# snsinfu/2022a-genome-dynamics

Hardware: AMD Instinct MI355X
Metric: bead-steps/sec on 100kb whole-genome model, 1 GPU and 8-GPU replica farm (higher is better)
Workload: dtype f32

## Files before the change

### 2022a-genome-dynamics_amd/__init__.py

```python
from __future__ import annotations

import ctypes as C
import os
from dataclasses import dataclass

import numpy as np

_HERE = os.path.dirname(os.path.abspath(__file__))
LIBGDYN_PATH = os.path.join(_HERE, "csrc", "libgdyn.so")

GD_BOX_OPEN, GD_BOX_PERIODIC = 0, 1
POT_HARMONIC, POT_SPRING, POT_SEMISPRING, POT_SOFTCORE = 0, 1, 2, 3
NOISE_PHILOX, NOISE_ZERO, NOISE_HOST, NOISE_MT19937 = 0, 1, 2, 3
RUN_UPDATE_SCALES, RUN_WALL_DYNAMICS, RUN_DEFER_CALLBACK, RUN_COMPENSATED, RUN_UNCOMPENSATED = 1, 2, 4, 8, 16
ALL_REPLICAS = 0xffffffff
ABI_VERSION = 5
TERM_PAIR, TERM_BOND, TERM_BEND, TERM_POINT, TERM_WALL, TERM_DYNAMIC, TERM_ALL = 1, 2, 4, 8, 16, 32, 63

_STATUS = {1: "GD_EINVAL", 2: "GD_ENODEVICE", 3: "GD_EHIP", 4: "GD_ENOMEM", 5: "GD_ESTATE", 6: "GD_EUNSUPPORTED"}


class GdynError(RuntimeError):
    def __init__(self, code, msg):
        super().__init__(f"{_STATUS.get(code, code)}: {msg}")
# ... 330 lines not shown

    def set_tuning(self, skin=0.0, rebuild_interval=0, adapt_interval=1, list_width=0, kernel_path=0, near_fraction=0.0, auto_skin=0):
        t = Tuning(skin, rebuild_interval, adapt_interval, list_width, kernel_path, near_fraction, auto_skin)
        self.lib.check(self.lib.dll.gd_set_tuning(self._h, C.byref(t)))

    def _groups_fn(self, name):
        f = getattr(self.lib.dll, name, None)
        if f is None:
            raise GdynError(6, f"{name}: not in this library (include/gdyn_groups.h: csrc/libgdyn.so only)")
        return f

    def set_step_groups(self, mode=0):
        f = self._groups_fn("gd_set_step_groups")
        f.argtypes = [C.c_void_p, C.c_uint32]
        self.lib.check(f(self._h, mode))

    def step_groups(self):
        f = self._groups_fn("gd_get_step_groups")
        f.argtypes = [C.c_void_p, C.POINTER(C.c_uint32), C.POINTER(C.c_uint32)]
        mode, last = C.c_uint32(0), C.c_uint32(0)
        self.lib.check(f(self._h, C.byref(mode), C.byref(last)))
        return mode.value, last.value

    def timing(self):
        t = Timing()
        self.lib.check(self.lib.dll.gd_get_timing(self._h, C.byref(t)))
        return t

    def debug_bench(self, what, n=20):
        f = getattr(self.lib.dll, "gd_debug_bench", None)
        if f is None:
            raise GdynError(6, "gd_debug_bench: not in this library (developer builds only: make -C csrc dev; load('libgdyn_dev.so'))")
        f.argtypes = [C.c_void_p, C.c_int, C.c_int, C.POINTER(C.c_double)]
        ms = C.c_double(0)
        self.lib.check(f(self._h, what, n, C.byref(ms)))
        return ms.value

    def stream(self):
        p = C.c_void_p()
        self.lib.check(self.lib.dll.gd_get_stream(self._h, C.byref(p)))
        return p.value
```

### 2022a-genome-dynamics_amd/csrc/gdyn_capi.hip

```cpp
#include <algorithm>
#include <cmath>
#include <cstdio>
#include <cstdlib>
#include <cstring>
#include <new>
#include <string>
#include <vector>

#include <hip/hip_fp16.h>

#include "gdyn_system.hpp"
#include "gdyn_once.hpp"
#ifdef GD_DEV
#include "gdyn_dev.h"
#endif


static thread_local char g_err[1024];
extern "C" const char *gd_last_error(void) { return g_err; }
int gd_report_error(int code, const char *msg)
{
    snprintf(g_err, sizeof g_err, "%s", msg);
    return code;
}
// ... 40 lines not shown
    if (s->R % GD_XCDS == 0 && !dev_env("GDYN_SLICE_MAP")) s->cpb = 0;
    s->ens.reset(s->N, s->R); s->mob.assign(s->N, 1.0); s->bend.assign(s->N, 0.0);
    s->hctx.assign(s->R, DevCtx{});
    for (auto &c : s->hctx) { c.bead_scale = 1; c.bond_scale = 1; }
    s->rp.reset(s->N, s->R);
    s->lcount.assign(2 * (size_t)s->R, 0ull);
    s->ncell_cap = (uint32_t)std::min<uint64_t>(std::max<uint64_t>(8ull * s->N, 4096ull), 262144ull);
    if (const char *e = dev_env("GDYN_NEAR_FRAC")) s->near_frac = atof(e);
    if (const char *e = dev_env("GDYN_SKIN")) { s->pol.skin = atof(e); s->pol.skin_fixed = true; }
    if (dev_env("GDYN_AUTO_SKIN")) s->pol.tuner.enabled = true;
    if (const char *e = dev_env("GDYN_TILE_CAPS")) { auto &c = s->pol.tile_caps; c.clear(); for (const char *q = e; *q;) { c.push_back((unsigned)strtoul(q, (char **)&q, 10)); if (*q == ',') q++; } }
    if (const char *e = dev_env("GDYN_K_TARGET")) s->pol.k_target = atof(e);
    if (dev_env("GDYN_DEBUG")) s->pol.trace = stderr;
    size_t free_b = 0, total_b = 0;
    if (hipMemGetInfo(&free_b, &total_b) == hipSuccess) s->pol.mem_total = total_b;
    hipError_t e = hipStreamCreateWithFlags(&s->stream, hipStreamNonBlocking);
    if (e != hipSuccess) { delete s; return fail(GD_EHIP, "hipStreamCreate failed: %s", hipGetErrorString(e)); }
    const size_t RNp = (size_t)s->R * s->Np, RN = (size_t)s->R * s->N;
    bool ok = true;
    for (int k = 0; k < 2; k++) {
        ok = ok && s->pos[k].resize(RNp) == hipSuccess && s->orig[k].resize(RNp) == hipSuccess && s->ctx[k].resize(s->R) == hipSuccess &&
             s->react_part[k].resize((size_t)s->R * s->nblk) == hipSuccess;
    }
    ok = ok && s->xb.resize(RNp) == hipSuccess && s->slot_of.resize(RN) == hipSuccess && s->bbox_enc.resize((size_t)2 * s->R * 6) == hipSuccess && s->bbox_w.resize((size_t)s->R * s->nblk * (GD_BLOCK / 64) * 6) == hipSuccess &&
         s->rank.resize(RNp) == hipSuccess && s->members.resize(RNp) == hipSuccess && s->cell_cnt.resize((size_t)s->R * (s->ncell_cap + 1)) == hipSuccess &&
         s->cell_start.resize((size_t)s->R * (s->ncell_cap + 1)) == hipSuccess && s->meta.resize(RNp) == hipSuccess &&
         s->flags.resize((size_t)s->R * GD_NFLAGS) == hipSuccess && s->bbox.resize((size_t)s->R * s->nblk * 6) == hipSuccess &&
         s->ab.resize(RNp) == hipSuccess && s->mobs.resize(RNp) == hipSuccess && s->grid.resize(s->R) == hipSuccess &&
         s->epart.resize((size_t)s->R * s->nblk) == hipSuccess &&
         s->lcount_d.resize(2 * (size_t)s->R) == hipSuccess && s->dmax.resize((size_t)s->R * GD_DMAX_STRIDE) == hipSuccess && s->fout.resize(RN) == hipSuccess && s->snap.resize(RN) == hipSuccess &&
         s->tiles.resize((size_t)s->R * s->nblk) == hipSuccess &&
         s->rec_x0.resize(RNp) == hipSuccess && s->rec_mo.resize(RNp) == hipSuccess && s->len_prev.resize((size_t)s->R * s->N) == hipSuccess &&
         s->wtab.resize(RNp / 64) == hipSuccess && s->need_prev.resize((size_t)s->R * s->N) == hipSuccess && s->pool.resize(4) == hipSuccess && s->rqueue.resize(RNp / 64) == hipSuccess &&
         s->lo.resize(RN) == hipSuccess;
    s->lo_valid = ok;
    if (!ok) { delete s; return fail(GD_ENOMEM, "gd_create: device allocation failed (%zu slots)", RNp); }
    gd_launch_identity(s->orig[0].p, s->slot_of.p, s->N, s->Np, s->R, s->stream);
    if (hipStreamSynchronize(s->stream) != hipSuccess) { delete s; return fail(GD_EHIP, "gd_create: identity kernel failed"); }
    *out = s;
    return GD_OK;
}

extern "C" int gd_destroy(gd_system *s)
{
    if (!s) return GD_OK;
    (void)hipSetDevice(s->device);
// ... 292 lines not shown
    if (t->near_fraction < 0 || t->near_fraction > 1) return fail(GD_EINVAL, "gd_set_tuning: near_fraction must be in [0,1]");
    HIPCHK(hipSetDevice(s->device));
    if (s->pol.set_tuning(t->skin, t->rebuild_interval, t->adapt_interval, t->list_width, t->auto_skin != 0 || dev_env("GDYN_AUTO_SKIN")))
        (void)s->nbr.resize(0);
    if (t->near_fraction > 0) s->near_frac = t->near_fraction;
    s->kernel_path = t->kernel_path;
    s->list.drop();
    return GD_OK;
}
extern "C" int gd_get_timing(gd_system *s, gd_timing *o) { if (!s || !o) return fail(GD_EINVAL, "gd_get_timing: NULL"); *o = s->timing; return GD_OK; }
extern "C" int gd_groups_abi_version(void) { return GD_GROUPS_ABI_VERSION; }
extern "C" int gd_set_step_groups(gd_system *s, uint32_t mode)
{
    if (!s) return fail(GD_EINVAL, "gd_set_step_groups: NULL system");
    if (mode > gd::STEP_GROUPS_TWO) return fail(GD_EINVAL, "gd_set_step_groups: mode must be 0 (rule), 1 (one launch) or 2 (two groups wherever results allow)");
    s->group_mode = mode;
    return GD_OK;
}
extern "C" int gd_get_step_groups(gd_system *s, uint32_t *mode, uint32_t *last_groups)
{
    if (!s) return fail(GD_EINVAL, "gd_get_step_groups: NULL system");
    if (mode) *mode = s->group_mode;
    if (last_groups) *last_groups = s->groups_last;
    return GD_OK;
}
extern "C" int gd_get_stream(gd_system *s, void **st) { if (!s || !st) return fail(GD_EINVAL, "gd_get_stream: NULL"); *st = (void *)s->stream; return GD_OK; }


static float pair_cutoff(const gd_system *s)
{
    double m = 0;
    if (s->has_pair) {
        if (s->pair.eps_a != 0 && s->pair.sigma_a > m) m = s->pair.sigma_a;
        if (s->pair.eps_b != 0 && s->pair.sigma_b > m) m = s->pair.sigma_b;
    }
    return (float)m;
}

static int finalize_topology(gd_system *s)
{
    if (!s->topo_dirty) return GD_OK;
    HIPCHK(hipSetDevice(s->device));
    const uint32_t N = s->N;
    std::vector<gd_bond_params> types = s->btypes;
    std::vector<int> terms = s->bterm;
    std::vector<Bond> all = s->bonds;
// ... 418 lines not shown
        q.scaling.from_host = 1;
        q.scaling.bead_next = scale_at(s, s->bs_init, s->bs_tau, time);
        q.scaling.bond_next = scale_at(s, s->bo_init, s->bo_tau, time);
    };
    size_t nev = 0;
    HIPCHK(hipEventRecord(get_event(s, nev++), s->stream));
    int64_t k = 0;
    c.on_search_list = s->list.valid && s->list.search_list;
    while (k < chunk) {
        if (!s->list.valid || s->list.steps_since_build >= s->pol.K) {
            s->pol.take_pending_skin(pair_cutoff(s));
            hipEvent_t e1 = get_event(s, nev++);
            GDCHK(enqueue_build(s, list_radius(s, run, (uint32_t)(k + s->pol.K)), with_list));
            s->list.enter_use(false);
            HIPCHK(hipEventRecord(e1, s->stream));
            c.spans.push_back({nev - 1, 1});
        }
        const int64_t n = std::min<int64_t>((int64_t)s->pol.K - s->list.steps_since_build, chunk - k);
        hipEvent_t e1 = get_event(s, nev++);
        uint32_t min_blocks = gd::STEP_GROUPS_MIN_BLOCKS, a16 = gd::STEP_GROUPS_A16;
        if (const char *e = dev_env("GDYN_GROUP_MIN_BLOCKS")) min_blocks = (uint32_t)atoi(e);
        if (const char *e = dev_env("GDYN_GROUP_A16")) a16 = (uint32_t)atoi(e);
        const uint32_t ra = gd::step_group_split(s->group_mode, group_state(s, host_noise), min_blocks, a16);
        if (ra) { GDCHK(fork_groups(s)); s->groups_last = 2; }
        for (int64_t q = 0; q < n; q++) {
            fill_common(s, p);
            p.dt_d = run->timestep; p.dt = (float)run->timestep; p.kT = (float)run->temperature; p.seed = run->seed;
            p.seeds = run->replica_seeds ? s->seeds_d.p : nullptr;
            p.noise_mode = run->noise_mode; p.run_flags = run->flags; p.comp = comp ? 1 : 0;
            p.host_noise = host_noise ? s->noise.p + (size_t)(done + k + q) * RN * 3 : nullptr;
            host_scales(p, k + q);
            p.record_disp = (s->list.steps_since_build + (uint32_t)q + 1u == s->pol.K);
            c.full_interval |= p.record_disp != 0;
            if (ra) {
                p.r0 = 0; p.nrep = ra; gd_launch_step(p, GD_MODE_STEP, s->stream);
                p.r0 = ra; p.nrep = s->R - ra; gd_launch_step(p, GD_MODE_STEP, s->stream2);
            } else gd_launch_step(p, GD_MODE_STEP, s->stream);
            if (s->sw.n) launch_softwell(s, p, 0);
            if (s->rp.any()) launch_replica_pairs(s, p, 0);
            s->pcur ^= 1; s->ccur ^= 1;
        }
        if (ra) GDCHK(join_groups(s));
        HIPCHK(hipEventRecord(e1, s->stream));
        c.spans.push_back({nev - 1, 0});
        s->timing.step_launches += (uint64_t)n;
        s->list.stepped((uint32_t)n);
        k += n;
    }
    const bool defer = (run->flags & GD_RUN_DEFER_CALLBACK) && done + chunk == run->steps;
    if (!defer) {
        fill_common(s, p);
        p.dt_d = run->timestep; p.dt = (float)run->timestep; p.run_flags = run->flags;
        host_scales(p, chunk);
        gd_launch_finalize(p, 0, s->stream);
        s->ccur ^= 1;
    } else {
        s->pend_dt = run->timestep; s->pend_flags = run->flags;
        if (s->has_wall) {
            fill_common(s, p);
// ... 50 lines not shown
    return GD_OK;
}

extern "C" int gd_run(gd_system *s, const gd_run_desc *run)
{
    if (!s || !run) return fail(GD_EINVAL, "gd_run: NULL argument");
    if (run->spacestep != 0) return fail(GD_EUNSUPPORTED, "gd_run: spacestep != 0 (adaptive timestep) is not supported");
    if (run->steps < 0 || !(run->timestep > 0) || run->temperature < 0) return fail(GD_EINVAL, "gd_run: bad steps/timestep/temperature");
    if (run->noise_mode < 0 || run->noise_mode > GD_NOISE_HOST)
        return fail(run->noise_mode == 3 ? GD_EUNSUPPORTED : GD_EINVAL, "gd_run: noise_mode %d not available on the device", run->noise_mode);
    if (run->noise_mode == GD_NOISE_HOST && !run->host_noise) return fail(GD_EINVAL, "gd_run: host noise requested without array");
    if ((run->flags & GD_RUN_WALL_DYNAMICS) && !s->has_wall) return fail(GD_ESTATE, "gd_run: wall dynamics requested without a wall");
    if ((run->flags & GD_RUN_UPDATE_SCALES) && !s->has_scaling) return fail(GD_ESTATE, "gd_run: scale updates requested without gd_set_scaling");
    GDCHK(prepare(s));
    GDCHK(apply_pending(s));
    s->state_serial++;
    if (run->timestep != s->last_dt || run->temperature != s->last_kT) { s->pol.a2_ema = 0; s->last_dt = run->timestep; s->last_kT = run->temperature; }
    if (s->pol.adapt && s->pol.K > 4 && ((run->flags ^ s->last_flags) & (GD_RUN_WALL_DYNAMICS | GD_RUN_UPDATE_SCALES)) != 0 && s->rebuilds > 0)
        s->pol.K -= s->pol.K / 5;
    s->last_flags = run->flags;
    const bool with_list = pair_cutoff(s) > 0;
    const size_t RN = (size_t)s->R * s->N;
    memset(&s->timing, 0, sizeof s->timing);
    s->groups_last = 1;

    const bool host_noise = run->noise_mode == GD_NOISE_HOST && run->temperature > 0;
    if (host_noise) {
        const size_t n = (size_t)run->steps * RN * 3;
        std::vector<float> h(n);
        for (size_t i = 0; i < n; i++) h[i] = (float)run->host_noise[i];
        HIPCHK(s->noise.resize(n, false));
        HIPCHK(hipMemcpy(s->noise.p, h.data(), n * sizeof(float), hipMemcpyHostToDevice));
    }

    const bool comp = run->steps > 0 && want_compensated(s, run);
    if (comp) {
        if (!s->lo_valid) { HIPCHK(hipMemsetAsync(s->lo.p, 0, RN * sizeof(float4), s->stream)); s->lo_valid = true; }
        HIPCHK(s->snap_lo.resize(RN, false));
    }
    if (run->steps > 0) s->comp_last = comp;
    if (run->steps > 0 && !comp) s->lo_valid = false;

    if (run->replica_seeds) {
        static_assert(sizeof(unsigned long long) == sizeof(uint64_t), "seed width");
        HIPCHK(s->seeds_d.resize(s->R, false));
        HIPCHK(hipMemcpy(s->seeds_d.p, run->replica_seeds, s->R * sizeof(uint64_t), hipMemcpyHostToDevice));
    }
// ... 178 lines not shown
```

### 2022a-genome-dynamics_amd/csrc/gdyn_kernels.hip

```cpp
#include <hip/hip_fp16.h>

#include <algorithm>

#include "gdyn_types.h"

#include "gdyn_stamps.h"

#if GD_ABL == 40 || GD_ABL == 41 || GD_ABL == 43
#define GD_REPLAY 1
constexpr bool RP_MEM = (GD_ABL == 40), RP_ALU = (GD_ABL == 41 || GD_ABL == 43);
#define GD_CONSUME4(v) asm volatile("" :: "v"((v).x), "v"((v).y), "v"((v).z), "v"((v).w))
#define GD_LAUNDER4(v) asm volatile("" : "+v"((v).x), "+v"((v).y), "+v"((v).z), "+v"((v).w))
#endif

#define TERM_PAIR 1u
#define TERM_BOND 2u
#define TERM_BEND 4u
#define TERM_POINT 8u
#define TERM_WALL 16u
#define TERM_DYNAMIC 32u
#define RUN_UPDATE_SCALES 1
#define RUN_WALL_DYNAMICS 2
#define NOISE_PHILOX 0
#define NOISE_ZERO 1
// ... 404 lines not shown
__device__ __forceinline__ float integrate(const StepParams &p, const CtxF &s_ctx, const StepBead &bead, unsigned r, unsigned blk,
                                           float mu, const float3 &z, const float3 &F, float disp2)
{
    const float3 xi = bead.xi;
    const float mu_dt = mu * p.dt;
    const float sg = s_ctx.sg_uniform >= 0.f ? s_ctx.sg_uniform : sqrtf(2.0f * p.kT * mu_dt);
    const float ex = mu_dt * F.x + sg * z.x, ey = mu_dt * F.y + sg * z.y, ez = mu_dt * F.z + sg * z.z;
    float nx = xi.x + ex, ny = xi.y + ey, nz = xi.z + ez;
    if (p.comp) {
        float4 *lp = p.lo + ((size_t)r * p.N + bead.oid);
        const float4 l = *lp;
        const float tx = l.x + ex, ty = l.y + ey, tz = l.z + ez;
        nx = xi.x + tx; ny = xi.y + ty; nz = xi.z + tz;
        const float bx = nx - xi.x, by = ny - xi.y, bz = nz - xi.z;
        *lp = make_float4((xi.x - (nx - bx)) + (tx - bx), (xi.y - (ny - by)) + (ty - by), (xi.z - (nz - bz)) + (tz - bz), 0.f);
    }
    if (TILED) *(float4 *)((char *)(p.pos_out + bead.rbase + (size_t)blk * GD_BLOCK) + bead.local * 16u) = make_float4(nx, ny, nz, bead.xi4.w);
    else p.pos_out[bead.g] = make_float4(nx, ny, nz, bead.xi4.w);
    float dnew2 = 0.f;
    if (TILED) { const float e2 = ex * ex + ey * ey + ez * ez; dnew2 = (disp2 + e2 + 2.0f * __builtin_amdgcn_sqrtf(disp2 * e2)) * 1.000002f; }
    return dnew2;
}

template <int MODE, bool PERIODIC, bool TILED, int PK, bool S16, bool SPLIT = false>
#ifndef GD_STEP_WAVES
#define GD_STEP_WAVES 8
#endif
__global__ __launch_bounds__(GD_BLOCK, (TILED && MODE == GD_MODE_STEP) ? (S16 ? GD_STEP_WAVES : 4) : 1) void k_step(const StepParams p)
{
    extern __shared__ __attribute__((aligned(16))) float4 s_tile[];
    __shared__ BondType s_bt[GD_MAX_BOND_TYPES];
    __shared__ CtxF s_ctx;
    __shared__ float s_red[GD_BLOCK / 64][4];
    __shared__ double s_e[GD_BLOCK / 64];

    unsigned r, blk;
    if (!block_map(blockIdx.x, p.nblk, p.cpb, r, blk)) return;
    if (MODE == GD_MODE_STEP && TILED && PK != 0) r += p.r0;
    if (TILED && SPLIT) {
        const unsigned held = p.tiles[(size_t)r * p.nblk + blk].total;
        if (held <= p.tile_lo || held > p.tile_hi) return;
    }
    const unsigned tid = threadIdx.x, lane = tid & 63, wid = tid >> 6;
    const size_t rbase = (size_t)r * p.Np;
    const float4 *__restrict__ rpos = p.pos_in + rbase;

    GD_STAMP_BEGIN();
    const long long ctx_step0 = p.ctx_in[r].step;
    const int ctx_pending0 = p.ctx_in[r].pending;
    const float dmax0 = (MODE == GD_MODE_STEP && TILED) ? __uint_as_float(p.dmax[r * GD_DMAX_STRIDE]) : 0.f;
    const size_t gw6 = (rbase + blk * GD_BLOCK) / 64 + (size_t)(unsigned)__builtin_amdgcn_readfirstlane((int)wid);
    const uint2 wrow = TILED ? p.wtab[gw6] : make_uint2(0u, 0u);
    const unsigned NCL = TILED ? wrow.y : p.W / 4, NCB = p.WB / 4;
    uint2 mo = make_uint2(0u, 0u);
    float4 rec = make_float4(0.f, 0.f, 0.f, 0.f);
    uint4 adj0 = make_uint4(0, 0, 0, 0), qa = adj0, qb = adj0;
    unsigned own_base = 0, tile_ok = 0;
    if (TILED) {
        const size_t tbase = rbase + (size_t)blk * GD_BLOCK;
        mo = *(const uint2 *)((const char *)(p.rec_mo + tbase) + tid * 8u);
        const TileDesc *td = p.tiles + (size_t)r * p.nblk + blk;
        unsigned tlen[GD_TILE_RANGES], tst[GD_TILE_RANGES];
#pragma unroll
        for (int k = 0; k < GD_TILE_RANGES; k++) { tlen[k] = td->len[k]; tst[k] = td->start[k]; }
        own_base = td->own_base; tile_ok = td->nranges;
        asm volatile("" : "+v"(mo.x), "+v"(mo.y));
        GD_STAMP(9);
        {
            constexpr bool W0_FREE = MODE == GD_MODE_STEP;
            const unsigned wq = (unsigned)__builtin_amdgcn_readfirstlane((int)((W0_FREE ? (wid == 0 ? 0x100000u : wid - 1u) : wid) * 64u));
            constexpr unsigned DMA_STRIDE = W0_FREE ? GD_BLOCK - 64u : GD_BLOCK;
            if (wid == 0 && lane < 2 * GD_MAX_BOND_TYPES)
                __builtin_amdgcn_global_load_lds((const __attribute__((address_space(1))) void *)((const uint4 *)p.btab + lane),
                                                 (__attribute__((address_space(3))) void *)s_bt, 16, 0, 0);
            unsigned base = 0;
#pragma unroll
#ifdef GD_REPLAY
            for (int k = 0; k < (RP_ALU ? 0 : GD_TILE_RANGES); base += tlen[k], k++) {
#else
            for (int k = 0; k < GD_TILE_RANGES; base += tlen[k], k++) {
#endif
                const unsigned len = tlen[k], st = tst[k];
                for (unsigned q0 = wq; q0 < len; q0 += DMA_STRIDE) {
                    if (q0 + lane < len)
                        __builtin_amdgcn_global_load_lds((const __attribute__((address_space(1))) void *)((const char *)(rpos + st + q0) + lane * 16u),
                                                         (__attribute__((address_space(3))) void *)(s_tile + base + q0), 16, 0, 0);
                }
            }
        }
        GD_STAMP(11);
        rec = *(const float4 *)((const char *)(p.rec_x0 + tbase) + tid * 16u);
#ifdef GD_REPLAY
        if (!RP_ALU)
#endif
        {
        adj0 = ((const uint4 *)p.badj)[gw6 * NCB * 64 + lane];
        qa = nt_load((const uint4 *)p.nbr16 + (size_t)wrow.x * 64 + lane);
// ... 23 lines not shown
    if (TILED) {
        local = (mo.x >> 12) & 0x1ffu; nAq = mo.x >> 21; nA = (nAq + 1u) >> 1; nB = mo.y >> 26;
        meta = mo.x & 0xfffu;
        oid = mo.y & GD_REC_ID_MASK;
    }
    float3 z = make_float3(0.f, 0.f, 0.f);
    auto draw_noise = [&]() {
#ifdef GD_REPLAY
        if (RP_MEM) return;
#endif
#if GD_ABL == 53
        if (MODE == GD_MODE_STEP) return;
#endif
        if (MODE == GD_MODE_STEP && (TILED ? oid != GD_REC_ID_MASK : valid) && p.kT > 0.f) {
            if (p.noise_mode == NOISE_PHILOX) {
                const long long step_now = ctx_step0 + (ctx_pending0 ? 1 : 0);
                z = p.seeds ? philox_normal3(p.seeds[r], oid, step_now + 1, 0u) : philox_normal3(p.seed, oid, step_now + 1, r);
            } else if (p.noise_mode == NOISE_HOST) {
                const float *h = p.host_noise + ((size_t)r * p.N + oid) * 3;
                z = make_float3(h[0], h[1], h[2]);
            }
        }
    };
    const bool noise_late = TILED && MODE == GD_MODE_STEP && wid == 0;
    if (!noise_late) draw_noise();
    GD_STAMP_USE3(z.x, z.y, z.z);
    GD_STAMP(10);
    if (wid == 0) {
        DevCtx c = p.ctx_in[r];
        if (MODE == GD_MODE_STEP) {
            if (c.pending) apply_callback(c, p, r, lane);
            if (lane == 0 && blk == 0) { DevCtx o = c; o.pending = 1; p.ctx_out[r] = o; }
        }
        if (lane == 0) fill_ctxf(s_ctx, c, p);
    }
    GD_STAMP(0);
    __syncthreads();
    GD_STAMP(1);
    if (noise_late) draw_noise();
    if (TILED) {
        valid = oid != GD_REC_ID_MASK;
        slot = valid ? blk * GD_BLOCK + local : p.N;
        g = rbase + slot;
        if (valid) {
#if GD_ABL == 41 || GD_ABL == 43
            xi4 = p.pos_in[g];
#else
            xi4 = tile_ok ? s_tile[own_base + local] : p.pos_in[g];
#endif
            x0 = rec;
            if (MODE == GD_MODE_STEP && p.mob_uniform < 0.f) mu = p.mob[g];
// ... 287 lines not shown
            for (int w = 0; w < GD_BLOCK / 64; w++) v += s_e[w];
            p.epart[(size_t)r * p.nblk + blk] = v;
        }
    }
}

__global__ __launch_bounds__(64) void k_ctx(const StepParams p, int mode)
{
    const unsigned r = blockIdx.x, lane = threadIdx.x;
    DevCtx c = p.ctx_in[r];
    if (mode == 1) {
        double rx = 0, ry = 0, rz = 0;
        for (unsigned b = lane; b < p.nblk; b += 64) {
            const float4 v = p.react_in[(size_t)r * p.nblk + b];
            rx += v.x; ry += v.y; rz += v.z;
        }
        c.react[0] = wave_sum_d(rx); c.react[1] = wave_sum_d(ry); c.react[2] = wave_sum_d(rz);
    } else if (c.pending) {
        apply_callback(c, p, r, lane);
    }
    if (lane == 0) p.ctx_out[r] = c;
}

typedef void (*StepKernel)(StepParams);
template <int MODE, bool SPLIT, bool PER, bool TIL, bool S16>
static StepKernel step_kernel_pk(int pk)
{
    return pk == 1 ? k_step<MODE, PER, TIL, 1, S16, SPLIT> : pk == 2 ? k_step<MODE, PER, TIL, 2, S16, SPLIT> : k_step<MODE, PER, TIL, 0, S16, SPLIT>;
}
template <int MODE, bool SPLIT>
static StepKernel tiled_step_kernel(bool periodic, int pk, bool s16)
{
    static_assert(!SPLIT || MODE == GD_MODE_STEP, "only stepping is split by tile class");
    if (periodic) return s16 ? step_kernel_pk<MODE, SPLIT, true, true, true>(pk) : step_kernel_pk<MODE, SPLIT, true, true, false>(pk);
    return s16 ? step_kernel_pk<MODE, SPLIT, false, true, true>(pk) : step_kernel_pk<MODE, SPLIT, false, true, false>(pk);
}
template <int MODE>
static StepKernel step_kernel(bool periodic, bool tiled, int pk, bool s16)
{
    if (tiled) return tiled_step_kernel<MODE, false>(periodic, pk, s16);
    return periodic ? step_kernel_pk<MODE, false, true, false, false>(pk) : step_kernel_pk<MODE, false, false, false, false>(pk);
}

template <int MODE>
static void launch_step_mode(const StepParams &p, hipStream_t st)
{
    const dim3 grid(p.cpb ? GD_XCDS * p.cpb * p.nrep : p.nrep * p.nblk), block(GD_BLOCK);
    const size_t lds = p.tiled ? (size_t)p.tile_cap * sizeof(float4) : 0;
    const bool s16 = p.tiled && gd_tile_s16(p.tile_cap);
    const unsigned split_at = !p.tiled ? 0u : (s16 && p.tile_cap > 3312u) ? 3312u : (!s16 && p.tile_cap > 5072u) ? 5072u : (!s16 && p.tile_cap > 3312u) ? 3312u : 0u;
    if (MODE == GD_MODE_STEP && split_at) {
        const StepKernel k = tiled_step_kernel<GD_MODE_STEP, true>(p.periodic, p.pk, s16);
        StepParams q = p;
        for (int half = 0; half < 2; half++) {
            q.tile_cap = half ? p.tile_cap : split_at; q.tile_lo = half ? split_at : 0u; q.tile_hi = half ? 0xffffffffu : split_at;
            hipLaunchKernelGGL(k, grid, block, (size_t)q.tile_cap * sizeof(float4), st, q);
        }
        return;
    }
    const StepKernel k = step_kernel<MODE>(p.periodic, p.tiled, p.pk, s16);
    hipLaunchKernelGGL(k, grid, block, lds, st, p);
}

void gd_launch_step(const StepParams &p, int mode, hipStream_t st)
{
    if (mode == GD_MODE_STEP) launch_step_mode<GD_MODE_STEP>(p, st);
    else if (mode == GD_MODE_FORCE) launch_step_mode<GD_MODE_FORCE>(p, st);
    else launch_step_mode<GD_MODE_ENERGY>(p, st);
}

void gd_launch_finalize(const StepParams &p, int mode, hipStream_t st)
{
    hipLaunchKernelGGL(k_ctx, dim3(p.R), dim3(64), 0, st, p, mode);
}


template <int CTRL, int ROW_MASK>
__device__ __forceinline__ float dppi(float v, float ident)
{
    return __int_as_float(__builtin_amdgcn_update_dpp(__float_as_int(ident), __float_as_int(v), CTRL, ROW_MASK, 0xf, false));
}
template <bool MAX>
__device__ __forceinline__ float wave_minmax(float v)
{
    const float id = MAX ? -INFINITY : INFINITY;
#define GD_MM(a, b) (MAX ? fmaxf(a, b) : fminf(a, b))
    v = GD_MM(v, (dppi<0x111, 0xf>(v, id))); v = GD_MM(v, (dppi<0x112, 0xf>(v, id))); v = GD_MM(v, (dppi<0x114, 0xf>(v, id)));
    v = GD_MM(v, (dppi<0x118, 0xf>(v, id))); v = GD_MM(v, (dppi<0x142, 0xa>(v, id))); v = GD_MM(v, (dppi<0x143, 0xc>(v, id)));
#undef GD_MM
    return __int_as_float(__builtin_amdgcn_readlane(__float_as_int(v), 63));
}
__global__ __launch_bounds__(GD_BLOCK) void k_bbox(const BuildParams p)
{
    __shared__ float s_lo[GD_BLOCK / 64][3], s_hi[GD_BLOCK / 64][3];
    const unsigned nb4 = (p.nblk + 3u) / 4u;
    const unsigned r = blockIdx.x / nb4, blk0 = (blockIdx.x % nb4) * 4u;
// ... 1256 lines not shown
{
    const unsigned nb = (unsigned)std::min<unsigned long long>((from.cap + 255ull) / 256ull, 4096ull);
    hipLaunchKernelGGL(k_ct_rehash, dim3(nb, R), dim3(256), 0, st, from, to);
}

void gd_launch_contacts_compact(const ContactTab &t, unsigned r, unsigned long long *keys_out, unsigned *vals_out, unsigned *n_out, hipStream_t st)
{
    const unsigned nb = (unsigned)std::min<unsigned long long>((t.cap + 255ull) / 256ull, 8192ull);
    hipLaunchKernelGGL(k_ct_compact, dim3(nb), dim3(256), 0, st, t, r, keys_out, vals_out, n_out);
}

hipError_t gd_kernels_init_device(void)
{
    hipError_t first = hipSuccess;
    auto set = [&](const void *f, int bytes) {
        const hipError_t e = hipFuncSetAttribute(f, hipFuncAttributeMaxDynamicSharedMemorySize, bytes);
        if (e != hipSuccess && first == hipSuccess) first = e;
    };
    for (auto pick : {tiled_step_kernel<GD_MODE_STEP, false>, tiled_step_kernel<GD_MODE_STEP, true>, tiled_step_kernel<GD_MODE_FORCE, false>,
                      tiled_step_kernel<GD_MODE_ENERGY, false>})
        for (int per = 0; per < 2; per++)
            for (int pk = 0; pk < 3; pk++)
                for (int s16 = 0; s16 < 2; s16++) set(reinterpret_cast<const void *>(pick(per != 0, pk, s16 != 0)), 128 * 1024);
    for (int per = 0; per < 2; per++)
        for (int s16 = 0; s16 < 2; s16++)
            for (int rep = 0; rep < 2; rep++) set(reinterpret_cast<const void *>(fill_kernel(per != 0, true, s16 != 0, rep != 0)), 128 * 1024);
    set(reinterpret_cast<const void *>(&k_softwell<0>), 64 * 1024);
    set(reinterpret_cast<const void *>(&k_softwell<1>), 64 * 1024);
    set(reinterpret_cast<const void *>(&k_softwell<2>), 64 * 1024);
    return first;
}


__global__ void k_gather_positions(const float4 *pos, const unsigned *slot_of, float4 *out, unsigned N, unsigned Np, int quantize)
{
    const unsigned r = blockIdx.y, o = blockIdx.x * blockDim.x + threadIdx.x;
    if (o >= N) return;
    float4 x = pos[(size_t)r * Np + slot_of[(size_t)r * N + o]];
    if (quantize) {
        x.x = rintf(x.x * 65536.0f) * (1.0f / 65536.0f);
        x.y = rintf(x.y * 65536.0f) * (1.0f / 65536.0f);
        x.z = rintf(x.z * 65536.0f) * (1.0f / 65536.0f);
    }
    out[(size_t)r * N + o] = x;
}

// ... 39 lines not shown
```

### 2022a-genome-dynamics_amd/csrc/gdyn_policy.hpp

```cpp
#pragma once
#include <algorithm>
#include <cmath>
#include <cstdint>
#include <cstdio>
#include <cstring>
#include <vector>

#include "gdyn_types.h"

namespace gd {

struct BuildReport {
    unsigned bits = 0;
    bool over = false, class_over = false, tile_over = false, violated = false;
    unsigned need_w = 0, need_t = 0, ncell = 0;
    float maxd2 = 0;
};

inline BuildReport summarize(const unsigned *flags, uint32_t R)
{
    BuildReport b;
    for (const unsigned *f = flags; f < flags + (size_t)R * GD_NFLAGS; f += GD_NFLAGS) {
        b.bits |= f[GD_FLAG_OVERFLOW]; b.tile_over |= f[GD_FLAG_TILE_OVERFLOW] != 0; b.violated |= f[GD_FLAG_VIOLATION] != 0;
        b.need_w = std::max(b.need_w, f[GD_FLAG_NEED_W]); b.need_t = std::max(b.need_t, f[GD_FLAG_NEED_TILE]); b.ncell = std::max(b.ncell, f[GD_FLAG_NCELL]);
// ... 33 lines not shown

enum : uint32_t { STEP_GROUPS_RULE = 0, STEP_GROUPS_ONE = 1, STEP_GROUPS_TWO = 2 };
struct StepGroupState {
    uint32_t R = 0, nblk = 0;
    bool tiled = false;
    bool post_step = false;
    bool device_noise = true;
    bool whole_replica_map = false;
    bool fast_pair = false;
};
constexpr uint32_t STEP_GROUPS_MIN_BLOCKS = 384u;
constexpr uint32_t STEP_GROUPS_A16 = 8u;
inline uint32_t step_group_split(uint32_t mode, const StepGroupState &st, uint32_t min_blocks = STEP_GROUPS_MIN_BLOCKS, uint32_t a16 = STEP_GROUPS_A16)
{
    if (mode != STEP_GROUPS_RULE && mode != STEP_GROUPS_TWO) return 0;
    if (!st.tiled || st.post_step || !st.device_noise || !st.whole_replica_map || !st.fast_pair) return 0;
    if (st.R < 2 * GD_XCDS || st.R % GD_XCDS != 0 || st.nblk == 0) return 0;
    a16 = std::min(std::max(a16, 1u), 15u);
    uint32_t ra = (uint32_t)(((uint64_t)st.R * a16 + 8u * GD_XCDS) / (16u * GD_XCDS)) * GD_XCDS;
    ra = std::min(std::max(ra, (uint32_t)GD_XCDS), st.R - GD_XCDS);
    const uint32_t small = std::min(ra, st.R - ra);
    if (mode == STEP_GROUPS_RULE && (uint64_t)small * st.nblk < min_blocks) return 0;
    return ra;
}

struct ListPolicy {
    std::vector<unsigned> tile_caps = {3312u, 4080u, 5072u, 8192u};
    double k_target = 0.90;
    FILE *trace = nullptr;
    size_t mem_total = 0;
    double skin = 0.75;
    bool skin_fixed = false;
    double skin_next = 0;
    double skin_dense_from = 0;
    bool dense_by_tile = false;
    uint32_t dense_budget = 0;
    uint32_t skin_streak = 0, skin_hold = 0;
    uint32_t K = 4, adapt = 1, K_bad = 0, K_bad_ttl = 0;
    double a2_ema = 0;
    uint32_t W = 0, tile_cap = 3312, tile_hold = 0;
    bool all_near = false;
    bool tiled_ok = true; uint32_t tiled_off = 0;
    uint32_t tiled_wait = 0, tiled_backoff = 8;
    uint32_t repair_wide = 0;
    uint32_t last_need_w = 0, last_need_t = 0;
    uint32_t ncell_seen = 0;
// ... 254 lines not shown
```

### 2022a-genome-dynamics_amd/csrc/gdyn_system.hpp

```cpp
#pragma once
#include <cstdint>
#include <cstring>
#include <vector>

#include "../../include/gdyn.h"
#include "../../include/gdyn_replica.h"
#include "../../include/gdyn_ensemble.h"
#include "../../include/gdyn_groups.h"
#include "../../include/gdyn_glue.h"

#include "gdyn_types.h"
#include "gdyn_analysis.hpp"
#include "gdyn_policy.hpp"
#include "gdyn_list.hpp"
#include "gdyn_live.hpp"
#include "gdyn_replica_pairs.hpp"
#include "gdyn_ensemble.hpp"

using gd::fail;

struct Bond { uint32_t i, j; int type; };
struct BendRange { uint32_t start, end; double energy; int per_bead; };
struct PointSource { int kind; double k, b, p[3]; std::vector<uint8_t> mask; };
struct DynSet { bool used = false; gd_bond_params p; std::vector<uint32_t> pairs; };

namespace gd {

struct Droplet {
    uint32_t n = 0; double eps = 0, decay = 1, cut = 0;
    dbuf<unsigned> targets; dbuf<double> esum;
};
// ... 74 lines not shown
    gd::dbuf<unsigned short> nbr16; gd::dbuf<TileDesc> tiles;
    gd::dbuf<float4> rec_x0; gd::dbuf<uint2> rec_mo; gd::dbuf<unsigned char> len_prev;
    gd::dbuf<uint2> wtab, rqueue; gd::dbuf<unsigned short> need_prev; gd::dbuf<unsigned> pool;
    gd::dbuf<float> bbox;
    gd::dbuf<float2> ab; gd::dbuf<float> mobs; gd::dbuf<float4> bendE; gd::dbuf<int4> chain;
    float mob_uniform = -1.f;
    gd::dbuf<GridP> grid; gd::dbuf<DevCtx> ctx[2]; gd::dbuf<float4> react_part[2]; gd::dbuf<double> epart;
    gd::dbuf<unsigned long long> lcount_d; gd::dbuf<float> noise;
    gd::dbuf<unsigned long long> seeds_d;
    gd::dbuf<unsigned> dmax;
    double last_dt = 0, last_kT = -1;
    int last_flags = 0;
    double pend_dt = 0; int pend_flags = 0;
    double near_frac = 0.65;
    uint64_t state_serial = 1;
    int ocur = 0;
    gd::dbuf<float4> lo, snap_lo;
    bool lo_valid = false;
    bool comp_last = false;
    double mob_max = 1.0;
    std::vector<hipEvent_t> events;
    hipStream_t stream2 = nullptr; hipEvent_t grp_fork = nullptr, grp_join = nullptr;
    uint32_t group_mode = gd::STEP_GROUPS_RULE, groups_last = 1;

    gd::Droplet sw;
    gd::ReplicaPairs rp;
    gd::ReplicaUpload rp_up;
    gd::Glue gl;
    gd::SearchCache sp;
    gd::ContactTables ct;

    ~gd_system()
    {
        for (auto e : events) (void)hipEventDestroy(e);
        if (grp_fork) (void)hipEventDestroy(grp_fork);
        if (grp_join) (void)hipEventDestroy(grp_join);
        if (stream2) (void)hipStreamDestroy(stream2);
        if (stream) (void)hipStreamDestroy(stream);
    }
};


template <class P>
static void set_box(const gd_system *s, P &p)
{
    p.periodic = s->box_kind == GD_BOX_PERIODIC;
// ... 19 lines not shown
```

### 2022a-genome-dynamics_amd/csrc/gdyn_types.h

```cpp
#pragma once
#include <hip/hip_runtime.h>
#include <stdint.h>

#ifndef GD_BLOCK
#define GD_BLOCK 512
#endif
#define GD_MAX_BOND_TYPES 16
#define GD_MAX_POINT_SOURCES 4
#define GD_ADJ_SHIFT 26
#define GD_ADJ_MASK ((1u << GD_ADJ_SHIFT) - 1u)
#define GD_ADJ_LOCAL 0x80000000u
#define GD_CHAIN_LOCAL 0x40000000
#define GD_TILE_RANGES 9
#define GD_XCDS 8
#define GD_REC_NOBEAD 0xffffffffu
#define GD_TILED_MAX_NEAR 8184u
#define GD_TILED_MAX_FAR 504u
#define GD_TILED_MAX_W (GD_TILED_MAX_NEAR + GD_TILED_MAX_FAR)
inline bool gd_tile_s16(unsigned tile_cap) { return tile_cap < 4096u; }
#define GD_REC_ID_MASK 0x03ffffffu
#define GD_DMAX_STRIDE 32u
#define GD_REPAIR_GRID 1024u
#define GD_UNROLL 8u

// ... 18 lines not shown
#define GD_TD_OWN 29

struct DevCtx {
    long long step;
    int pending;
    int pad;
    double time, bead_scale, bond_scale;
    double semi[3];
    double react[3];
};

struct CtxF {
    long long step;
    float bead_scale, bond_scale, semi[3];
    float inv_semi[3], inv_semi2[3];
    float inv_bond_scale2;
    float near2;
    float w_inv_sa2, w_inv_sb2, w_ca, w_cb;
    float p_inv_sa2, p_inv_sb2, p_cut;
    float sg_uniform;
    float w_inv_q3;
    double w_q[4];
};

struct GridP {
    float org[3];
    float inv[3];
    int nc[3];
    int ncell;
};

struct PairP {
    float eps_a, sigma_a, eps_b, sigma_b;
    int p_a, q_a, p_b, q_b;
    int mix, scaled, enabled;
    float cutoff;
};

struct WallP {
    float eps_a, sigma_a, eps_b, sigma_b;
    int p_a, q_a, p_b, q_b;
    float wall_a, wall_b;
    int scaled, enabled;
    int fast2383;
    float packing_spring;
    double spring[3], mobility;
// ... 64 lines not shown
    WallP wall;
    ScaleP scaling;
    const BondType *btab;
    int nbt;
    PointSrc ps[GD_MAX_POINT_SOURCES];
    int nps;
    int has_bend, has_bonds;
    double dt_d;
    float dt, kT;
    unsigned long long seed;
    const unsigned long long *seeds;
    int noise_mode, run_flags;
    const float *host_noise;
    float rv;
    float rn;
    unsigned *dmax;
    int record_disp;
    unsigned nrep;
    float4 *lo;
    int comp;
    unsigned term_mask;
    float4 *fout;
    double *epart;
};

struct BuildParams {
    unsigned N, Np, R, nblk;
    size_t stride;
    int periodic;
    float box[3], inv_box[3];
    float rv;
    float rn;
    unsigned *dmax;
    unsigned ncell_cap;
    unsigned scan_segments;
    int kx;
    const float4 *pos_in;
    float4 *pos_out;
    float4 *xb;
    const unsigned *orig_in;
    unsigned *orig_out;
    unsigned *slot_of;
    unsigned *rank;
    unsigned *members;
    unsigned *cell_cnt, *cell_start;
    float *bbox;
// ... 22 lines not shown
    unsigned W;
    int tiled, packed_ab;
    int w_valid;
    unsigned cpb, tile_cap;
    unsigned *flags;
    unsigned long long *lcount;
    float4 *rec_x0; uint2 *rec_mo;
    unsigned char *len_prev;
    uint2 *wtab;
    unsigned short *need_prev;
    unsigned *pool;
    uint2 *rqueue;
    unsigned rq_cap;
    unsigned rq_grid;
    unsigned pool_cap;
    int predict;
    unsigned long long *dbg;
    unsigned ab_stride;
};

hipError_t gd_kernels_init_device(void);
void gd_launch_step(const StepParams &p, int mode, hipStream_t st);
void gd_launch_finalize(const StepParams &p, int mode, hipStream_t st);
void gd_launch_build(const BuildParams &p, hipStream_t st);
struct SoftwellP {
    const float4 *pos_in;
    float4 *pos_out;
    float4 *fout;
    double *esum;
    const unsigned *slot_of, *targets;
    const float *mob_o;
    float mob_uniform, dt, eps, inv_d2, rc2;
    float4 *lo;
    int comp;
    unsigned N, Np, R, M;
    int periodic;
    float box[3], inv_box[3];
};
void gd_launch_softwell(const SoftwellP &p, int mode, hipStream_t st);
#define GD_RP_SLOT_SHIFT 30
#define GD_RP_PARTNER_MASK ((1u << GD_RP_SLOT_SHIFT) - 1u)
struct ReplicaPairsP {
    const float4 *pos_in;
    float4 *pos_out, *fout;
    double *esum;
    const unsigned *slot_of;
// ... 49 lines not shown
```

Baseline: 25.85 billion.

## Precompute per-replica step context in a small kernel before grouped step launches

When stepping is split into two replica groups on two streams, a tiny per-replica kernel now applies pending callbacks and fills the CtxF context into a device buffer before each group's step kernel. A PREP specialisation of the tiled step kernel then DMA-loads the prepared context into LDS instead of having wave 0 compute it inline, so wave 0 can join tile staging and draw noise early. The aim is to shorten the step kernel's serial prologue, at the cost of two extra launches per step and more kernel instantiations. A heuristic on group size decides when this path is used.

Result: faster. 26.87 billion (median of 6 runs) (+3.9%).

```diff
diff --git a/2022a-genome-dynamics_amd/__init__.py b/2022a-genome-dynamics_amd/__init__.py
--- a/2022a-genome-dynamics_amd/__init__.py
+++ b/2022a-genome-dynamics_amd/__init__.py
@@ -376,6 +376,15 @@
         self.lib.check(f(self._h, C.byref(mode), C.byref(last)))
         return mode.value, last.value
 
+    def ctx_prepared(self):
+        f = getattr(self.lib.dll, "gd_get_ctx_prepared", None)
+        if f is None:
+            raise GdynError(6, "gd_get_ctx_prepared: not in this library (include/gdyn_prep.h: csrc/libgdyn.so only)")
+        f.argtypes = [C.c_void_p, C.POINTER(C.c_uint64)]
+        n = C.c_uint64(0)
+        self.lib.check(f(self._h, C.byref(n)))
+        return n.value
+
     def timing(self):
         t = Timing()
         self.lib.check(self.lib.dll.gd_get_timing(self._h, C.byref(t)))
diff --git a/2022a-genome-dynamics_amd/csrc/gdyn_capi.hip b/2022a-genome-dynamics_amd/csrc/gdyn_capi.hip
--- a/2022a-genome-dynamics_amd/csrc/gdyn_capi.hip
+++ b/2022a-genome-dynamics_amd/csrc/gdyn_capi.hip
@@ -86,6 +86,7 @@
         ok = ok && s->pos[k].resize(RNp) == hipSuccess && s->orig[k].resize(RNp) == hipSuccess && s->ctx[k].resize(s->R) == hipSuccess &&
              s->react_part[k].resize((size_t)s->R * s->nblk) == hipSuccess;
     }
+    ok = ok && s->ctxf.resize(s->R) == hipSuccess;
     ok = ok && s->xb.resize(RNp) == hipSuccess && s->slot_of.resize(RN) == hipSuccess && s->bbox_enc.resize((size_t)2 * s->R * 6) == hipSuccess && s->bbox_w.resize((size_t)s->R * s->nblk * (GD_BLOCK / 64) * 6) == hipSuccess &&
          s->rank.resize(RNp) == hipSuccess && s->members.resize(RNp) == hipSuccess && s->cell_cnt.resize((size_t)s->R * (s->ncell_cap + 1)) == hipSuccess &&
          s->cell_start.resize((size_t)s->R * (s->ncell_cap + 1)) == hipSuccess && s->meta.resize(RNp) == hipSuccess &&
@@ -424,6 +425,13 @@
     if (!s) return fail(GD_EINVAL, "gd_get_step_groups: NULL system");
     if (mode) *mode = s->group_mode;
     if (last_groups) *last_groups = s->groups_last;
+    return GD_OK;
+}
+extern "C" int gd_prep_abi_version(void) { return GD_PREP_ABI_VERSION; }
+extern "C" int gd_get_ctx_prepared(gd_system *s, uint64_t *launches)
+{
+    if (!s) return fail(GD_EINVAL, "gd_get_ctx_prepared: NULL system");
+    if (launches) *launches = s->prep_last;
     return GD_OK;
 }
 extern "C" int gd_get_stream(gd_system *s, void **st) { if (!s || !st) return fail(GD_EINVAL, "gd_get_stream: NULL"); *st = (void *)s->stream; return GD_OK; }
@@ -888,6 +896,10 @@
         if (const char *e = dev_env("GDYN_GROUP_MIN_BLOCKS")) min_blocks = (uint32_t)atoi(e);
         if (const char *e = dev_env("GDYN_GROUP_A16")) a16 = (uint32_t)atoi(e);
         const uint32_t ra = gd::step_group_split(s->group_mode, group_state(s, host_noise), min_blocks, a16);
+        uint32_t prep_mode = gd::CTX_PREP_RULE, prep_min_blocks = gd::CTX_PREP_MIN_BLOCKS;
+        if (const char *e = dev_env("GDYN_CTX_PREP")) prep_mode = (uint32_t)atoi(e);
+        if (const char *e = dev_env("GDYN_CTX_PREP_MIN_BLOCKS")) prep_min_blocks = (uint32_t)atoi(e);
+        const bool prepared = gd::ctx_prepared(s->group_mode, ra, group_state(s, host_noise), prep_mode, prep_min_blocks);
         if (ra) { GDCHK(fork_groups(s)); s->groups_last = 2; }
         for (int64_t q = 0; q < n; q++) {
             fill_common(s, p);
@@ -899,8 +911,14 @@
             p.record_disp = (s->list.steps_since_build + (uint32_t)q + 1u == s->pol.K);
             c.full_interval |= p.record_disp != 0;
             if (ra) {
-                p.r0 = 0; p.nrep = ra; gd_launch_step(p, GD_MODE_STEP, s->stream);
-                p.r0 = ra; p.nrep = s->R - ra; gd_launch_step(p, GD_MODE_STEP, s->stream2);
+                if (prepared) p.ctxf = s->ctxf.p;
+                p.r0 = 0; p.nrep = ra;
+                if (prepared) gd_launch_ctx_prep(p, s->stream);
+                gd_launch_step(p, GD_MODE_STEP, s->stream);
+                p.r0 = ra; p.nrep = s->R - ra;
+                if (prepared) gd_launch_ctx_prep(p, s->stream2);
+                gd_launch_step(p, GD_MODE_STEP, s->stream2);
+                if (prepared) s->prep_last += 2;
             } else gd_launch_step(p, GD_MODE_STEP, s->stream);
             if (s->sw.n) launch_softwell(s, p, 0);
             if (s->rp.any()) launch_replica_pairs(s, p, 0);
@@ -997,7 +1015,7 @@
     const bool with_list = pair_cutoff(s) > 0;
     const size_t RN = (size_t)s->R * s->N;
     memset(&s->timing, 0, sizeof s->timing);
-    s->groups_last = 1;
+    s->groups_last = 1; s->prep_last = 0;
 
     const bool host_noise = run->noise_mode == GD_NOISE_HOST && run->temperature > 0;
     if (host_noise) {
diff --git a/2022a-genome-dynamics_amd/csrc/gdyn_kernels.hip b/2022a-genome-dynamics_amd/csrc/gdyn_kernels.hip
--- a/2022a-genome-dynamics_amd/csrc/gdyn_kernels.hip
+++ b/2022a-genome-dynamics_amd/csrc/gdyn_kernels.hip
@@ -450,7 +450,10 @@
     return dnew2;
 }
 
-template <int MODE, bool PERIODIC, bool TILED, int PK, bool S16, bool SPLIT = false>
+template <int MODE, bool PERIODIC, bool TILED, int PK, bool S16, bool SPLIT = false, bool PREP = false>
+#ifndef GD_PREP_W0_STAGES
+#define GD_PREP_W0_STAGES 1
+#endif
 #ifndef GD_STEP_WAVES
 #define GD_STEP_WAVES 8
 #endif
@@ -458,8 +461,9 @@
 {
     extern __shared__ __attribute__((aligned(16))) float4 s_tile[];
     __shared__ BondType s_bt[GD_MAX_BOND_TYPES];
-    __shared__ CtxF s_ctx;
+    __shared__ __attribute__((aligned(16))) CtxF s_ctx;
     __shared__ float s_red[GD_BLOCK / 64][4];
+    static_assert(!PREP || (MODE == GD_MODE_STEP && TILED && PK != 0), "prepared contexts: tiled stepping with a specialised pair form only");
     __shared__ double s_e[GD_BLOCK / 64];
 
     unsigned r, blk;
@@ -495,12 +499,15 @@
         asm volatile("" : "+v"(mo.x), "+v"(mo.y));
         GD_STAMP(9);
         {
-            constexpr bool W0_FREE = MODE == GD_MODE_STEP;
+            constexpr bool W0_FREE = MODE == GD_MODE_STEP && !(PREP && GD_PREP_W0_STAGES);
             const unsigned wq = (unsigned)__builtin_amdgcn_readfirstlane((int)((W0_FREE ? (wid == 0 ? 0x100000u : wid - 1u) : wid) * 64u));
             constexpr unsigned DMA_STRIDE = W0_FREE ? GD_BLOCK - 64u : GD_BLOCK;
             if (wid == 0 && lane < 2 * GD_MAX_BOND_TYPES)
                 __builtin_amdgcn_global_load_lds((const __attribute__((address_space(1))) void *)((const uint4 *)p.btab + lane),
                                                  (__attribute__((address_space(3))) void *)s_bt, 16, 0, 0);
+            if (PREP && wid == 0 && lane < sizeof(CtxF) / 16u)
+                __builtin_amdgcn_global_load_lds((const __attribute__((address_space(1))) void *)((const uint4 *)(p.ctxf + r) + lane),
+                                                 (__attribute__((address_space(3))) void *)&s_ctx, 16, 0, 0);
             unsigned base = 0;
 #pragma unroll
 #ifdef GD_REPLAY
@@ -570,11 +577,11 @@
             }
         }
     };
-    const bool noise_late = TILED && MODE == GD_MODE_STEP && wid == 0;
+    const bool noise_late = TILED && MODE == GD_MODE_STEP && !PREP && wid == 0;
     if (!noise_late) draw_noise();
     GD_STAMP_USE3(z.x, z.y, z.z);
     GD_STAMP(10);
-    if (wid == 0) {
+    if (!PREP && wid == 0) {
         DevCtx c = p.ctx_in[r];
         if (MODE == GD_MODE_STEP) {
             if (c.pending) apply_callback(c, p, r, lane);
@@ -908,18 +915,33 @@
     if (lane == 0) p.ctx_out[r] = c;
 }
 
+__global__ __launch_bounds__(64) void k_ctx_prep(const StepParams p)
+{
+    const unsigned r = p.r0 + blockIdx.x, lane = threadIdx.x;
+    DevCtx c = p.ctx_in[r];
+    if (c.pending) apply_callback(c, p, r, lane);
+    if (lane == 0) {
+        DevCtx o = c; o.pending = 1; p.ctx_out[r] = o;
+        CtxF f;
+        fill_ctxf(f, c, p);
+        p.ctxf[r] = f;
+    }
+}
+
 typedef void (*StepKernel)(StepParams);
-template <int MODE, bool SPLIT, bool PER, bool TIL, bool S16>
+template <int MODE, bool SPLIT, bool PER, bool TIL, bool S16, bool PREP = false>
 static StepKernel step_kernel_pk(int pk)
 {
-    return pk == 1 ? k_step<MODE, PER, TIL, 1, S16, SPLIT> : pk == 2 ? k_step<MODE, PER, TIL, 2, S16, SPLIT> : k_step<MODE, PER, TIL, 0, S16, SPLIT>;
-}
-template <int MODE, bool SPLIT>
+    if constexpr (PREP) return pk == 1 ? k_step<MODE, PER, TIL, 1, S16, SPLIT, true> : k_step<MODE, PER, TIL, 2, S16, SPLIT, true>;
+    else return pk == 1 ? k_step<MODE, PER, TIL, 1, S16, SPLIT> : pk == 2 ? k_step<MODE, PER, TIL, 2, S16, SPLIT> : k_step<MODE, PER, TIL, 0, S16, SPLIT>;
+}
+template <int MODE, bool SPLIT, bool PREP = false>
 static StepKernel tiled_step_kernel(bool periodic, int pk, bool s16)
 {
     static_assert(!SPLIT || MODE == GD_MODE_STEP, "only stepping is split by tile class");
-    if (periodic) return s16 ? step_kernel_pk<MODE, SPLIT, true, true, true>(pk) : step_kernel_pk<MODE, SPLIT, true, true, false>(pk);
-    return s16 ? step_kernel_pk<MODE, SPLIT, false, true, true>(pk) : step_kernel_pk<MODE, SPLIT, false, true, false>(pk);
+    static_assert(!PREP || MODE == GD_MODE_STEP, "only stepping runs on prepared contexts");
+    if (periodic) return s16 ? step_kernel_pk<MODE, SPLIT, true, true, true, PREP>(pk) : step_kernel_pk<MODE, SPLIT, true, true, false, PREP>(pk);
+    return s16 ? step_kernel_pk<MODE, SPLIT, false, true, true, PREP>(pk) : step_kernel_pk<MODE, SPLIT, false, true, false, PREP>(pk);
 }
 template <int MODE>
 static StepKernel step_kernel(bool periodic, bool tiled, int pk, bool s16)
@@ -935,8 +957,9 @@
     const size_t lds = p.tiled ? (size_t)p.tile_cap * sizeof(float4) : 0;
     const bool s16 = p.tiled && gd_tile_s16(p.tile_cap);
     const unsigned split_at = !p.tiled ? 0u : (s16 && p.tile_cap > 3312u) ? 3312u : (!s16 && p.tile_cap > 5072u) ? 5072u : (!s16 && p.tile_cap > 3312u) ? 3312u : 0u;
+    const bool prep = MODE == GD_MODE_STEP && p.ctxf != nullptr;
     if (MODE == GD_MODE_STEP && split_at) {
-        const StepKernel k = tiled_step_kernel<GD_MODE_STEP, true>(p.periodic, p.pk, s16);
+        const StepKernel k = prep ? tiled_step_kernel<GD_MODE_STEP, true, true>(p.periodic, p.pk, s16) : tiled_step_kernel<GD_MODE_STEP, true>(p.periodic, p.pk, s16);
         StepParams q = p;
         for (int half = 0; half < 2; half++) {
             q.tile_cap = half ? p.tile_cap : split_at; q.tile_lo = half ? split_at : 0u; q.tile_hi = half ? 0xffffffffu : split_at;
@@ -944,7 +967,8 @@
         }
         return;
     }
-    const StepKernel k = step_kernel<MODE>(p.periodic, p.tiled, p.pk, s16);
+    StepKernel k = step_kernel<MODE>(p.periodic, p.tiled, p.pk, s16);
+    if constexpr (MODE == GD_MODE_STEP) { if (prep) k = tiled_step_kernel<GD_MODE_STEP, false, true>(p.periodic, p.pk, s16); }
     hipLaunchKernelGGL(k, grid, block, lds, st, p);
 }
 
@@ -958,6 +982,11 @@
 void gd_launch_finalize(const StepParams &p, int mode, hipStream_t st)
 {
     hipLaunchKernelGGL(k_ctx, dim3(p.R), dim3(64), 0, st, p, mode);
+}
+
+void gd_launch_ctx_prep(const StepParams &p, hipStream_t st)
+{
+    hipLaunchKernelGGL(k_ctx_prep, dim3(p.nrep), dim3(64), 0, st, p);
 }
 
 
@@ -2260,6 +2289,10 @@
         for (int per = 0; per < 2; per++)
             for (int pk = 0; pk < 3; pk++)
                 for (int s16 = 0; s16 < 2; s16++) set(reinterpret_cast<const void *>(pick(per != 0, pk, s16 != 0)), 128 * 1024);
+    for (auto pick : {tiled_step_kernel<GD_MODE_STEP, false, true>, tiled_step_kernel<GD_MODE_STEP, true, true>})
+        for (int per = 0; per < 2; per++)
+            for (int pk = 1; pk < 3; pk++)
+                for (int s16 = 0; s16 < 2; s16++) set(reinterpret_cast<const void *>(pick(per != 0, pk, s16 != 0)), 128 * 1024);
     for (int per = 0; per < 2; per++)
         for (int s16 = 0; s16 < 2; s16++)
             for (int rep = 0; rep < 2; rep++) set(reinterpret_cast<const void *>(fill_kernel(per != 0, true, s16 != 0, rep != 0)), 128 * 1024);
diff --git a/2022a-genome-dynamics_amd/csrc/gdyn_policy.hpp b/2022a-genome-dynamics_amd/csrc/gdyn_policy.hpp
--- a/2022a-genome-dynamics_amd/csrc/gdyn_policy.hpp
+++ b/2022a-genome-dynamics_amd/csrc/gdyn_policy.hpp
@@ -79,6 +79,16 @@
     const uint32_t small = std::min(ra, st.R - ra);
     if (mode == STEP_GROUPS_RULE && (uint64_t)small * st.nblk < min_blocks) return 0;
     return ra;
+}
+
+enum : uint32_t { CTX_PREP_NEVER = 0, CTX_PREP_RULE = 1, CTX_PREP_ALWAYS = 2 };
+constexpr uint32_t CTX_PREP_MIN_BLOCKS = 1888u;
+inline bool ctx_prepared(uint32_t group_mode, uint32_t ra, const StepGroupState &st, uint32_t prep = CTX_PREP_RULE, uint32_t min_blocks = CTX_PREP_MIN_BLOCKS)
+{
+    if (ra == 0 || ra >= st.R || prep == CTX_PREP_NEVER) return false;
+    if (prep == CTX_PREP_ALWAYS || group_mode == STEP_GROUPS_TWO) return true;
+    if (group_mode != STEP_GROUPS_RULE) return false;
+    return (uint64_t)std::min(ra, st.R - ra) * st.nblk >= min_blocks;
 }
 
 struct ListPolicy {
diff --git a/2022a-genome-dynamics_amd/csrc/gdyn_system.hpp b/2022a-genome-dynamics_amd/csrc/gdyn_system.hpp
--- a/2022a-genome-dynamics_amd/csrc/gdyn_system.hpp
+++ b/2022a-genome-dynamics_amd/csrc/gdyn_system.hpp
@@ -7,6 +7,7 @@
 #include "../../include/gdyn_replica.h"
 #include "../../include/gdyn_ensemble.h"
 #include "../../include/gdyn_groups.h"
+#include "../../include/gdyn_prep.h"
 #include "../../include/gdyn_glue.h"
 
 #include "gdyn_types.h"
@@ -127,6 +128,8 @@
     std::vector<hipEvent_t> events;
     hipStream_t stream2 = nullptr; hipEvent_t grp_fork = nullptr, grp_join = nullptr;
     uint32_t group_mode = gd::STEP_GROUPS_RULE, groups_last = 1;
+    gd::dbuf<CtxF> ctxf;
+    uint64_t prep_last = 0;
 
     gd::Droplet sw;
     gd::ReplicaPairs rp;
diff --git a/2022a-genome-dynamics_amd/csrc/gdyn_types.h b/2022a-genome-dynamics_amd/csrc/gdyn_types.h
--- a/2022a-genome-dynamics_amd/csrc/gdyn_types.h
+++ b/2022a-genome-dynamics_amd/csrc/gdyn_types.h
@@ -64,6 +64,7 @@
     float w_inv_q3;
     double w_q[4];
 };
+static_assert(sizeof(CtxF) % 16 == 0 && sizeof(CtxF) <= 64 * 16, "CtxF is copied into LDS in 16-byte pieces by one wave");
 
 struct GridP {
     float org[3];
@@ -174,6 +175,7 @@
     unsigned term_mask;
     float4 *fout;
     double *epart;
+    CtxF *ctxf;
 };
 
 struct BuildParams {
@@ -242,6 +244,7 @@
 hipError_t gd_kernels_init_device(void);
 void gd_launch_step(const StepParams &p, int mode, hipStream_t st);
 void gd_launch_finalize(const StepParams &p, int mode, hipStream_t st);
+void gd_launch_ctx_prep(const StepParams &p, hipStream_t st);
 void gd_launch_build(const BuildParams &p, hipStream_t st);
 struct SoftwellP {
     const float4 *pos_in;
diff --git a/include/gdyn_prep.h b/include/gdyn_prep.h
--- /dev/null
+++ b/include/gdyn_prep.h
@@ -0,0 +1,21 @@
+#ifndef GDYN_PREP_H
+#define GDYN_PREP_H
+
+#include <stdint.h>
+
+#include "gdyn.h"
+
+#ifdef __cplusplus
+extern "C" {
+#endif
+
+#define GD_PREP_ABI_VERSION 1
+
+int gd_prep_abi_version(void);
+int gd_get_ctx_prepared(gd_system *sys, uint64_t *launches);
+
+#ifdef __cplusplus
+}
+#endif
+
+#endif
```
